# octavian-ganea/equidock_public

Hardware: NVIDIA H100
Metric: protein_pairs_per_sec_iegmn_fwd_kabsch (higher is better)
Workload: dtype f32

## Files before the change

### equidock_public_b200/_native.py

```python
from __future__ import annotations

import ctypes as C
import os

_HERE = os.path.dirname(os.path.abspath(__file__))
LIB_PATH = os.environ.get('EQD_LIB_PATH') or os.path.join(_HERE, 'libeqd_iegmn.so')

ABI_VERSION = 15
EDGE_FEATS, N_RBF, HID, H0, H0_PAD, N_RES_TYPES, HEADS, TILE_ROWS = 27, 15, 64, 69, 72, 21, 50, 128
MAX_HEADS = 64
STATUS_SVD_DEGENERATE, STATUS_NAN, STATUS_DEGREE_OVERFLOW, STATUS_BAD_RESIDUE = 1, 2, 4, 8

_vp, _i32, _f32 = C.c_void_p, C.c_int32, C.c_float


class EqdGraph(C.Structure):
    _fields_ = [('n_pairs', _i32), ('n_nodes', _i32), ('n_lig_nodes', _i32), ('n_edges', _i32),
                ('n_lig_edges', _i32), ('max_in_degree', _i32),
                ('seg_ptr', _vp), ('row_ptr', _vp), ('col_src', _vp), ('edge_dst', _vp),
                ('he_lig', _vp), ('he_rec', _vp),
                ('n_node_tiles', _i32), ('node_tiles', _vp)]


class EqdLayerParams(C.Structure):
    _fields_ = [('dh', _i32), ('dhp', _i32),
                ('w_proj', _vp), ('b_proj', _vp), ('w_edge1', _vp), ('edge_ln_g', _vp), ('edge_ln_b', _vp),
                ('w_edge2', _vp), ('b_edge2', _vp), ('w_coor1', _vp), ('b_coor1', _vp), ('w_coor2', _vp),
                ('b_coor2', _f32), ('w_edge_tc', _vp), ('w_node_tc', _vp), ('w_proj_tc', _vp),
                ('w_node1', _vp), ('b_node1', _vp), ('node_ln_g', _vp), ('node_ln_b', _vp),
                ('w_node2', _vp), ('b_node2', _vp),
                ('skip_weight_h', _f32), ('x_connection_init', _f32), ('leaky_slope', _f32), ('mma_products', _i32)]


class EqdLayerConsts(C.Structure):
    _fields_ = [('edge', _f32 * 64 * 5), ('node', _f32 * 304), ('proj_bias', _f32 * 320)]


class EqdDropout(C.Structure):
    _fields_ = [('seed', C.c_uint64), ('p', _f32), ('scale', _f32), ('threshold', C.c_uint32), ('layer', _i32),
                ('rank', _i32), ('reserved', _i32)]


def dropout_descriptor(p: float, seed: int, layer: int, rank: int = 0) -> EqdDropout:
    import numpy as np
    d = EqdDropout()
    d.seed, d.p, d.layer, d.rank = int(seed) & 0xFFFFFFFFFFFFFFFF, float(p), int(layer), int(rank)
    d.threshold = min(int(round(float(p) * 2.0 ** 32)), 0xFFFFFFFF)
    d.scale = 0.0 if p >= 1.0 else float(np.float32(1.0 / (1.0 - float(p))))
    return d


class EqdLayerNorms(C.Structure):
    _fields_ = [('coors_ln_g', _vp), ('coors_ln_b', _vp), ('final_ln_g', _vp), ('final_ln_b', _vp)]


class EqdLayer(C.Structure):
    _fields_ = [('dev', EqdLayerParams), ('consts', EqdLayerConsts), ('dropout', EqdDropout), ('norms', EqdLayerNorms)]


class EqdForwardIO(C.Structure):
    _fields_ = [(n, _vp) for n in ('emb', 'res_lig', 'res_rec', 'mu_lig', 'mu_rec', 'x_lig', 'x_rec', 'rot', 'trans',
                                   'ligand_out', 'sing', 'status', 'h_out', 'x_out', 'keypts', 'cov', 'ymean', 'stage_events',
                                   'train_stash')] + \
               [('train_stash_bytes', C.c_size_t)]


class EqdHeadParams(C.Structure):
    _fields_ = [('w_mean', _vp), ('b_mean', _vp), ('w_key', _vp), ('w_query', _vp), ('m_qk', _vp), ('leaky_slope', _f32),
                ('n_heads', _i32)]


class EqdPairArchive(C.Structure):
    _fields_ = [('n_pairs', _i32)] + [(n, _vp) for n in (
        'lig_node_ptr', 'rec_node_ptr', 'lig_edge_ptr', 'rec_edge_ptr', 'pocket_ptr', 'lig_res_feat', 'rec_res_feat',
        'lig_x', 'rec_x', 'lig_mu_r_norm', 'rec_mu_r_norm', 'lig_src', 'lig_dst', 'rec_src', 'rec_dst', 'lig_he', 'rec_he',
        'lig_new_x', 'pocket_coors', 'bound_lig', 'bound_rec', 'lig_centroid')]


class EqdBatchOut(C.Structure):
    _fields_ = [(n, _vp) for n in ('res_feat', 'x', 'new_x', 'mu_r_norm', 'row_ptr', 'col_src', 'edge_dst', 'he_lig', 'he_rec',
                                   'seg_ptr',
                                   'node_tiles', 'pocket_ptr', 'pocket_lig', 'pocket_rec', 'bound_lig', 'bound_rec', 'rot',
                                   'trans')]


_G, _L, _H = C.POINTER(EqdGraph), C.POINTER(EqdLayer), C.POINTER(EqdHeadParams)
PROTOTYPES = {
    'eqd_abi_version': (C.c_int, []),
    'eqd_workspace_bytes': (C.c_size_t, [_i32, _i32, _i32]),
    'eqd_workspace_bytes_k': (C.c_size_t, [_i32, _i32, _i32, _i32]),
    'eqd_embed': (C.c_int, [_G, _vp, _vp, _vp, _vp, _vp, _vp, _vp, _vp, _vp, _vp]),
    'eqd_embed_checked': (C.c_int, [_G, _vp, _vp, _vp, _vp, _vp, _vp, _vp, _vp, _vp, _vp, _vp]),
    'eqd_project': (C.c_int, [_G, _L, _vp, _i32, _vp, _vp]),
    'eqd_edge_stage': (C.c_int, [_G, _L, _vp, _vp, _vp, _vp, _vp, _vp, _vp]),
    'eqd_edge_stage_ffma': (C.c_int, [_G, _L, _vp, _vp, _vp, _vp, _vp, _vp, _vp]),
    'eqd_node_stage': (C.c_int, [_G, _L, _L, _vp, _i32, _vp, _vp, _vp, _vp, _vp, _vp, _vp]),
    'eqd_kv_blocks_bytes': (C.c_size_t, [_i32]),
    'eqd_project_tc': (C.c_int, [_G, _L, _vp, _vp, _vp, _vp]),
    'eqd_project_tc0': (C.c_int, [_G, _L, _vp, _vp, _vp, _vp, _vp]),
    'eqd_attention_tc0': (C.c_int, [_G, _vp, _vp, _vp, _vp, _vp]),
    'eqd_node_mlp_tc0': (C.c_int, [_G, _L, _vp, _vp, _vp, _vp, _vp]),
    'eqd_node_stage_tc0': (C.c_int, [_G, _L, _L, _vp, _vp, _vp, _vp, _vp, _vp, _vp, _vp, _vp]),
    'eqd_kv_blocks': (C.c_int, [_G, _vp, _i32, _i32, _i32, _vp, _vp]),
    'eqd_attention_tc': (C.c_int, [_G, _vp, _vp, _vp, _vp]),
    'eqd_node_mlp_tc': (C.c_int, [_G, _L, _vp, _vp, _vp, _vp, _vp, _vp]),
    'eqd_node_stage_tc': (C.c_int, [_G, _L, _L, _vp, _vp, _vp, _vp, _vp, _vp, _vp, _vp, _vp]),
    'eqd_iegmn_layer_forward': (C.c_int, [_G, _L, _L, _vp, _i32, _vp, _vp, _vp, _vp, _vp, _vp, _vp, _vp, _vp, _vp,
                                          _vp]),
    'eqd_head_fold': (C.c_int, [_H, _vp, _vp]),
    'eqd_forward_workspace_bytes': (C.c_size_t, [_G]),
    'eqd_forward_workspace_bytes_k': (C.c_size_t, [_G, _i32]),
    'eqd_iegmn_forward': (C.c_int, [_G, C.POINTER(_L), _i32, _H, C.POINTER(EqdForwardIO), _vp, C.c_size_t, _vp]),
    'eqd_forward_stash_bytes': (C.c_size_t, [_G, _i32]),
    'eqd_forward_stash_offsets': (C.c_int, [_G, _i32, C.POINTER(C.c_size_t)]),
    'eqd_tn_partial_floats': (C.c_size_t, [C.c_int64, _i32, _i32, C.POINTER(_i32), C.POINTER(_i32)]),
    'eqd_tn_gemm': (C.c_int, [_vp, _i32, _i32, _vp, _i32, _i32, C.c_int64, _f32, _vp, _vp, C.POINTER(_i32), _vp]),
    'eqd_grad_reduce': (C.c_int, [_vp, _i32, C.c_int64, _vp, _vp, _i32, _vp, _vp]),
    'eqd_bwd_node_mlp': (C.c_int, [_G, _L] + [_vp] * 3 + [_i32, _vp, _vp, _i32] + [_vp] * 9 + [C.POINTER(_i32), _vp]),
    'eqd_bwd_attention': (C.c_int, [_G, _L, _vp, _vp, _i32, _vp, _vp, _vp, _vp]),
    'eqd_bwd_edge': (C.c_int, [_G, _L] + [_vp] * 14 + [C.POINTER(_i32), _vp]),
    'eqd_bwd_edge_gather': (C.c_int, [_G, _vp, _vp, _vp, _vp, _vp, _f32, _vp, _i32, _vp, _vp]),
    'eqd_bwd_project': (C.c_int, [_G, _L, _vp, _vp, _vp, _vp]),
    'eqd_bwd_embed': (C.c_int, [_G, _vp, _vp, _vp, _vp, _vp, _vp]),
    'eqd_bwd_head_workspace_bytes': (C.c_size_t, [_i32, _i32, _i32]),
    'eqd_bwd_head_workspace_bytes_k': (C.c_size_t, [_i32, _i32, _i32, _i32]),
    'eqd_bwd_head': (C.c_int, [_G, _H] + [_vp] * 9 + [C.c_size_t] + [_vp] * 6),
    'eqd_bwd_head_dropout': (C.c_int, [_G, _H, C.POINTER(EqdDropout)] + [_vp] * 9 + [C.c_size_t] + [_vp] * 6),
    'eqd_bwd_layer_inputs': (C.c_int, [_G, _L] + [_vp] * 5),
    'eqd_bwd_inputs': (C.c_int, [_G] + [_vp] * 11),
    'eqd_losses_workspace_bytes': (C.c_size_t, [_i32, _i32]),
    'eqd_losses': (C.c_int, [_G] + [_vp] * 7 + [_i32, _i32, _f32, _f32, _f32, _f32, _vp, C.c_size_t] + [_vp] * 6),
    'eqd_losses_workspace_bytes_k': (C.c_size_t, [_i32, _i32, _i32]),
    'eqd_losses_k': (C.c_int, [_G] + [_vp] * 4 + [_i32] + [_vp] * 3 + [_i32, _i32, _f32, _f32, _f32, _f32, _vp, C.c_size_t] +
                     [_vp] * 6),
    'eqd_graph_build_workspace_bytes': (C.c_size_t, [_i32]),
    'eqd_graph_build_knn': (C.c_int, [_i32, _i32, _i32, _vp, _vp, _vp, _vp, _vp, _f32, _i32, _vp, C.c_size_t, _vp, _vp, _vp, _vp]),
    'eqd_graph_build_edges': (C.c_int, [_i32, _vp, _vp, _vp, _vp, _vp, _vp, _vp]),
    'eqd_assemble_batch': (C.c_int, [C.POINTER(EqdPairArchive), _i32, _vp, _i32, C.c_uint64, C.c_uint64, _i32, _f32, _i32,
                                     C.POINTER(EqdBatchOut), _vp]),
    'eqd_rmsd_meter': (C.c_int, [_G, _vp, _vp, _vp, _vp, _vp, _vp]),
    'eqd_sqnorm_partials': (C.c_int, [_vp, C.c_int64, _vp, _i32, _vp]),
    'eqd_clip_adam': (C.c_int, [_vp, _vp, _vp, _vp, C.c_int64, _vp, _i32, _f32, _f32, _f32, _f32, _f32, _f32, _i32, _f32, _vp, _vp]),
    'eqd_event_create': (_vp, []),
    'eqd_event_destroy': (None, [_vp]),
    'eqd_event_elapsed_ms': (C.c_float, [_vp, _vp]),
    'eqd_keypoints': (C.c_int, [_G, _H, _vp, _vp, _vp, C.c_size_t, _vp, _vp, _vp, _vp]),
    'eqd_keypoints_dropout': (C.c_int, [_G, _H, C.POINTER(EqdDropout), _vp, _vp, _vp, C.c_size_t, _vp, _vp, _vp, _vp]),
    'eqd_kabsch_apply': (C.c_int, [_G, _vp, _vp, _vp, _vp, _vp, _vp, _vp, _vp, _vp, _vp]),
}

_lib = None


class NativeLibraryError(RuntimeError):
    pass


def load():
    global _lib
    if _lib is not None:
        return _lib
    if not os.path.isfile(LIB_PATH):
        raise NativeLibraryError(
            f'{LIB_PATH} not found: build it with equidock_public_b200/csrc/build.sh '
            '(python -c "import __graft_entry__ as g; g.build()"). This engine has no CPU fallback.')
    lib = C.CDLL(LIB_PATH)
    for name, (res, args) in PROTOTYPES.items():
        fn = getattr(lib, name)
        fn.restype, fn.argtypes = res, args
    if lib.eqd_abi_version() != ABI_VERSION:
        raise NativeLibraryError(f'ABI mismatch: library {lib.eqd_abi_version()} vs binding {ABI_VERSION}')
    _lib = lib
    return lib

# ... 15 lines not shown
```

### equidock_public_b200/csrc/attn_tc.cu

```cuda
#include "tc_common.cuh"

namespace eqd {

#define AT_THREADS 256
#define AT_KEYS 64
#define AT_CHUNK_BYTES 8192
#define AT_A_SPLIT 16384
#define AT_LD 68

struct AtGroupSmem {
  unsigned char k[2][3][AT_CHUNK_BYTES];
  unsigned char v[2][3][AT_CHUNK_BYTES];
  float red[EQD_TM * 2];
  float x5c[2][AT_KEYS * 16];
  float red5[EQD_TM * 2 * 5];
};
struct AtSmem {
  unsigned char qa[3 * AT_A_SPLIT];
  unsigned char pa[3 * AT_A_SPLIT];
  AtGroupSmem grp;
  unsigned long long k_bar[2], v_bar[2];
};

__global__ void __launch_bounds__(AT_THREADS, 1)
// ... 235 lines not shown
      m.j0 = __ldg(g.seg_ptr + pseg);
      m.j1 = __ldg(g.seg_ptr + pseg + 1);
      m.blk_lo = m.j0 >> 3;
      m.nchunks = (((m.j1 + 7) >> 3) - m.blk_lo + 7) >> 3;
      return k;
    }
    return -1;
  };
  unsigned kfill = 0, kcons = 0, vfill = 0, vcons = 0;
  auto fill = [&](unsigned char (*dst)[3][AT_CHUNK_BYTES], unsigned long long* bars, unsigned& n, const unsigned char* src,
                  int blk0) {
    if (t == 0) {
      unsigned long long* b = &bars[n & 1];
      mbar_expect_tx(b, 3 * AT_CHUNK_BYTES);
#pragma unroll
      for (int s = 0; s < 3; ++s) bulk_g2s(dst[n & 1][s], src + s * kv_split_stride + (long)blk0 * 1024, AT_CHUNK_BYTES, b);
    }
    ++n;
  };
  auto consume = [&](unsigned long long* bars, unsigned& n) {
    mbar_wait(&bars[n & 1], (n >> 1) & 1);
    return (int)((n++) & 1);
  };
  auto stage_q = [&](const AtTile& m) { stage_rows64(W.qs, proj, 320, 128, m.node0, m.nvalid, t); };

  const int fr0 = (t >> 5) * 16 + (lane >> 2), fc = 2 * (lane & 3);
  AtTile cur, nxt;
  int kt = find_tile(0, cur);
  bool k_ahead = false, v_ahead = false;
  if (kt >= 0) stage_q(cur);
  while (kt >= 0) {
    int ktn = -1;
    bool looked = false;
    auto look_ahead = [&]() {
      if (looked) return;
      looked = true;
      ktn = find_tile(kt + 1, nxt);
      if (ktn >= 0) stage_q(nxt);
    };
    if (cur.nchunks > 0 && !k_ahead) fill(W.k, W.k_bar, kfill, k_g, cur.blk_lo);
    cp_async_wait<0>();
    wg_barrier(bar);
    unsigned qf[3][4][4];
    staged_rows_to_a_split3<P>(W.qs, t, qf);
    wg_barrier(bar);
    auto k_desc = [&](int kb_) {
      return [&, kb_](int sp, int kk) { return b_desc_ex(k_saddr + (kb_ * 3 + sp) * AT_CHUNK_BYTES + kk * 256, 128, 1024); };
    };
    float mx[2] = {-INFINITY, -INFINITY};
    for (int c = 0; c < cur.nchunks; ++c) {
      const int kb_ = consume(W.k_bar, kcons);
      fill(W.k, W.k_bar, kfill, k_g, cur.blk_lo + (c + 1 < cur.nchunks ? 8 * (c + 1) : 0));
      float s[32];
      wg_gemm6_rs_issue<64, 4, 0, true>(s, qf, k_desc(kb_), false);
      look_ahead();
      wg_mma_wait(s);
      const int key0 = (cur.blk_lo + 8 * c) * 8 + fc;
#pragma unroll
      for (int j = 0; j < 8; ++j)
#pragma unroll
        for (int e = 0; e < 2; ++e) {
          const int kn = key0 + 8 * j + e;
          const bool ok = kn >= cur.j0 && kn < cur.j1;
#pragma unroll
          for (int h = 0; h < 2; ++h) mx[h] = fmaxf(mx[h], ok ? s[4 * j + 2 * h + e] : -INFINITY);
        }
      wg_barrier(bar);
    }
    look_ahead();
#pragma unroll
    for (int h = 0; h < 2; ++h) {
      mx[h] = fmaxf(mx[h], __shfl_xor_sync(0xffffffffu, mx[h], 1));
      mx[h] = fmaxf(mx[h], __shfl_xor_sync(0xffffffffu, mx[h], 2));
    }
    float lh[2][2] = {{0.f, 0.f}, {0.f, 0.f}};
    float o_acc[32];
#pragma unroll
    for (int i = 0; i < 32; ++i) o_acc[i] = 0.f;
    if (cur.nchunks > 0 && !v_ahead) fill(W.v, W.v_bar, vfill, v_g, cur.blk_lo);
    for (int c = 0; c < cur.nchunks; ++c) {
      const int kb_ = consume(W.k_bar, kcons);
      const bool last = c + 1 == cur.nchunks;
      if (!last) {
        fill(W.k, W.k_bar, kfill, k_g, cur.blk_lo + 8 * (c + 1));
        fill(W.v, W.v_bar, vfill, v_g, cur.blk_lo + 8 * (c + 1));
      } else if (ktn >= 0 && nxt.nchunks > 0) {
        fill(W.k, W.k_bar, kfill, k_g, nxt.blk_lo);
        fill(W.v, W.v_bar, vfill, v_g, nxt.blk_lo);
      }
      float s[32];
      wg_gemm6_rs_issue<64, 4, 0, false, P>(s, qf, k_desc(kb_), false);
      wg_mma_wait(s);
      const int key0 = (cur.blk_lo + 8 * c) * 8 + fc;
#pragma unroll
      for (int j = 0; j < 8; ++j)
#pragma unroll
        for (int e = 0; e < 2; ++e) {
          const int kn = key0 + 8 * j + e;
          const bool ok = kn >= cur.j0 && kn < cur.j1;
#pragma unroll
          for (int h = 0; h < 2; ++h) {
            float& x = s[4 * j + 2 * h + e];
            x = ok ? expf(x - mx[h]) : 0.f;
          }
        }
      {
        float ps[32];
#pragma unroll
        for (int i = 0; i < 32; ++i) ps[i] = __shfl_xor_sync(0xffffffffu, s[i], 2);
#pragma unroll
        for (int h = 0; h < 2; ++h)
#pragma unroll
          for (int ch = 0; ch < 2; ++ch) {
            float s0 = 0.f, s1 = 0.f;
#pragma unroll
            for (int c4 = 0; c4 < 8; ++c4) {
              s0 = __fadd_rn(s0, chain_val(s, ps, h, ch, c4, 0));
              s1 = __fadd_rn(s1, chain_val(s, ps, h, ch, c4, 1));
            }
            const float sp = __fadd_rn(s0, s1);
            lh[h][ch] = __fadd_rn(lh[h][ch], __fadd_rn(sp, __shfl_xor_sync(0xffffffffu, sp, 1)));
          }
      }
      unsigned pf[3][4][4];
      acc_to_a_split3<4, P>(s, pf);
      const int vb_ = consume(W.v_bar, vcons);
      float o[32];
      wg_gemm6_rs_issue<64, 4, 1, false, P>(o, pf, [&](int sp, int kk) {
        return b_desc_ex(v_saddr + (vb_ * 3 + sp) * AT_CHUNK_BYTES + kk * 2048, 1024, 128); }, false);
      wg_mma_wait(o);
#pragma unroll
      for (int i = 0; i < 32; ++i) o_acc[i] = __fadd_rn(o_acc[i], o[i]);
      wg_barrier(bar);
    }
    k_ahead = v_ahead = ktn >= 0 && nxt.nchunks > 0 && cur.nchunks > 0;
#pragma unroll
    for (int h = 0; h < 2; ++h) {
      const float l = __fadd_rn(lh[h][0], lh[h][1]);
      const float inv = l > 0.f ? 1.f / l : 0.f;
      const int row = fr0 + 8 * h;
      if (row < cur.nvalid) {
        float* dst = mu + (long)(cur.node0 + row) * EQD_HID + fc;
#pragma unroll
        for (int j = 0; j < 8; ++j)
          *reinterpret_cast<float2*>(dst + 8 * j) = make_float2(o_acc[4 * j + 2 * h] * inv, o_acc[4 * j + 2 * h + 1] * inv);
      }
    }
    kt = ktn;
    cur = nxt;
  }
  cp_async_wait<0>();
}

template <int P>
static int launch_attention64_tc(const eqd_graph* g, const float* proj, const void* kv, float* mu, void* stream) {
  const size_t smem = AT_CHAINS * sizeof(AtChainSmem);
  EQD_SET_SMEM(attention64_tc_kernel<P>, smem);
  const int nht = 2 * g->n_node_tiles;
  int grid = (nht + AT_CHAINS - 1) / AT_CHAINS;
  if (grid > EQD_SMS) grid = EQD_SMS;
  const long split_stride = (long)((g->n_nodes + 7) / 8 + 8) * 1024;
  attention64_tc_kernel<P><<<grid, AT_CHAINS * 128, smem, (cudaStream_t)stream>>>(
      *g, proj, reinterpret_cast<const unsigned char*>(kv), split_stride, mu);
  EQD_CUDA_LAUNCH_CHECK();
  return EQD_OK;
}

}

int eqd_attention_tc_products(const eqd_graph* g, const float* proj, const void* kv, float* mu, int products, void* stream) {
  if (!g || !proj || !kv || !mu) return EQD_ERR_BAD_ARG;
  if (reinterpret_cast<uintptr_t>(kv) & 15) return EQD_ERR_BAD_ARG;
  if (products != 6 && products != 3) return EQD_ERR_UNSUPPORTED;
  if (g->n_node_tiles <= 0) return EQD_OK;
  return products == 3 ? eqd::launch_attention64_tc<3>(g, proj, kv, mu, stream)
                       : eqd::launch_attention64_tc<6>(g, proj, kv, mu, stream);
}

extern "C" int eqd_attention_tc(const eqd_graph* g, const float* proj, const void* kv, float* mu, void* stream) {
  return eqd_attention_tc_products(g, proj, kv, mu, 6, stream);
}

extern "C" int eqd_attention_tc0(const eqd_graph* g, const float* proj, const void* kv, const float* x5, float* mu,
                                 void* stream) {
  if (!g || !proj || !kv || !x5 || !mu) return EQD_ERR_BAD_ARG;
  if ((reinterpret_cast<uintptr_t>(kv) | reinterpret_cast<uintptr_t>(x5)) & 15) return EQD_ERR_BAD_ARG;
  if (g->n_node_tiles <= 0) return EQD_OK;
  const size_t smem = sizeof(eqd::AtSmem) + 128;
  EQD_SET_SMEM(eqd::attention0_tc_kernel, smem);
  const int grid = g->n_node_tiles < EQD_SMS ? g->n_node_tiles : EQD_SMS;
  const long split_stride = (long)((g->n_nodes + 7) / 8 + 8) * 1024;
  eqd::attention0_tc_kernel<<<grid, AT_THREADS, smem, (cudaStream_t)stream>>>(
      *g, proj, 128 + 3 * 72, reinterpret_cast<const unsigned char*>(kv), split_stride, x5, mu, EQD_H0_PAD);
  EQD_CUDA_LAUNCH_CHECK();
  return EQD_OK;
}
```

### equidock_public_b200/engine.py

```python
from __future__ import annotations

import ctypes as C
import sys
import threading
from typing import Dict, List, Optional, Sequence

import numpy as np
import torch

from . import _native as nat
from .hetero_graph import LIGAND, LL, RECEPTOR, RR


def _dev_f32(t, device):
    return t.detach().to(device=device, dtype=torch.float32).contiguous()


def _host_f32(t):
    return t.detach().to(device='cpu', dtype=torch.float32).contiguous()


def _upload_blob(tensors: Dict[str, torch.Tensor], device) -> Dict[str, torch.Tensor]:
    offs, total = {}, 0
    for k, t in tensors.items():
# ... 128 lines not shown
            w5p[:69, 80:144] = w5[:, 69:133]
            w5p[:69, 144:213] = w5[:, 133:202]
            tc['w_node_tc'] = torch.cat([umma_bf16x3(w5p), umma_bf16x3(p80(w6).contiguous())]).contiguous()
            assert tc['w_proj_tc'].numel() * 2 == 161280 and tc['w_node_tc'].numel() * 2 == 138240
            p80v = lambda v: torch.cat([v, z(80 - v.shape[0])])
            self.node_consts_host = torch.cat([p80v(b5), p80v(f('node_mlp.3.weight')), p80v(f('node_mlp.3.bias')), b6]).cpu().contiguous()
            pb = z(320)
            pb[64:128] = b1
            self.proj_bias_host = pb.cpu().contiguous()
        self.t = _upload_blob({
            **tc,
            'w_proj': w_proj, 'b_proj': b_proj, 'w_edge1': w_edge1,
            'edge_ln_g': f('edge_mlp.3.weight'), 'edge_ln_b': f('edge_mlp.3.bias'),
            'w_edge2': f('edge_mlp.4.weight').t().contiguous(), 'b_edge2': f('edge_mlp.4.bias'),
            'w_coor1': f('coors_mlp.0.weight').t().contiguous(), 'b_coor1': f('coors_mlp.0.bias'),
            'w_coor2': f('coors_mlp.4.weight').reshape(-1).contiguous(),
            'w_node1': w_node1, 'b_node1': pad(b5),
            'node_ln_g': pad(f('node_mlp.3.weight')), 'node_ln_b': pad(f('node_mlp.3.bias')),
            'w_node2': w_node2, 'b_node2': b6, 'w_edge_tc': w_edge_tc,
            **({'_coors_ln_g': f('coors_mlp.3.weight'), '_coors_ln_b': f('coors_mlp.3.bias')}
               if layer_norm_coors == 'LN' else {}),
            **({'_final_ln_g': f('final_h_layernorm_layer.weight'), '_final_ln_b': f('final_h_layernorm_layer.bias')}
               if final_h_layer_norm == 'LN' else {}),
        }, device)
        lay = nat.EqdLayer()
        s = lay.dev
        s.dh, s.dhp = dh, dhp
        for k, v in self.t.items():
            if not k.startswith('_'):
                setattr(s, k, v.data_ptr())
        for name, host in (('edge', self.edge_consts_host), ('node', self.node_consts_host), ('proj_bias', self.proj_bias_host)):
            if host is not None:
                flat = host.reshape(-1).numpy()
                C.memmove(C.addressof(getattr(lay.consts, name)), flat.ctypes.data, flat.nbytes)
        s.b_coor2 = float(sd['coors_mlp.4.bias'].detach().reshape(-1)[0].item())
        s.skip_weight_h, s.x_connection_init, s.leaky_slope = skip_weight_h, x_connection_init, leaky_slope
        if layer_norm_coors == 'LN':
            lay.norms.coors_ln_g, lay.norms.coors_ln_b = self.t['_coors_ln_g'].data_ptr(), self.t['_coors_ln_b'].data_ptr()
        if final_h_layer_norm == 'LN':
            lay.norms.final_ln_g, lay.norms.final_ln_b = self.t['_final_ln_g'].data_ptr(), self.t['_final_ln_b'].data_ptr()
        self.struct = lay
        self._descriptors = {}

    def descriptor(self, mma_products: int = 0):
        if mma_products == 0 or self.dh != nat.HID:
            return self.struct
        src, d = self._descriptors.get(mma_products, (None, None))
        if src is not self.struct:
            d = nat.EqdLayer.from_buffer_copy(self.struct)
            d.dev.mma_products = mma_products
            self._descriptors[mma_products] = (self.struct, d)
        return d


class PackedHead:

    def __init__(self, w_mean, b_mean, w_key, w_query, device, leaky_slope: float):
        dev = torch.device(device)
        inplace = all(t.is_cuda and t.device == dev and t.dtype == torch.float32 and t.is_contiguous() and t.data_ptr() % 16 == 0
                      for t in (b_mean, w_key, w_query)) and w_mean.is_cuda
        if inplace:
            self.t = {'w_mean': w_mean.detach().to(torch.float32).t().contiguous(), 'b_mean': b_mean.detach(),
                      'w_key': w_key.detach(), 'w_query': w_query.detach()}
        else:
            self.t = _upload_blob({'w_mean': _host_f32(w_mean).t().contiguous(), 'b_mean': _host_f32(b_mean),
                                   'w_key': _host_f32(w_key), 'w_query': _host_f32(w_query)}, device)
        self.n_heads = self.t['w_key'].shape[0] // nat.HID
        assert 1 <= self.n_heads <= nat.MAX_HEADS and self.t['w_key'].shape == (self.n_heads * nat.HID, nat.HID)
        assert self.t['w_query'].shape == self.t['w_key'].shape
        s = nat.EqdHeadParams()
        for k, v in self.t.items():
            if not k.startswith('_'):
                setattr(s, k, v.data_ptr())
        s.leaky_slope = leaky_slope
        s.n_heads = self.n_heads
        self.struct = s
        self.m_qk = torch.empty(self.n_heads, nat.HID, nat.HID, dtype=torch.float64, device=device)
        with torch.cuda.device(device):
            nat.check(nat.load().eqd_head_fold(C.byref(s), self.m_qk.data_ptr(), torch.cuda.current_stream().cuda_stream),
                      'eqd_head_fold')
        s.m_qk = self.m_qk.data_ptr()


def _aligned_he(he, device):
    he = he.to(device=device, dtype=torch.float32).contiguous()
    nbytes = he.numel() * 4
    try:
        room = he.untyped_storage().nbytes() - he.storage_offset() * 4
    except RuntimeError:
        room = nbytes
    if he.data_ptr() % 16 == 0 and room >= ((nbytes + 15) & ~15):
        return he
    buf = torch.empty(((nbytes + 15) // 16) * 4 + 4, dtype=torch.float32, device=device)
    own = buf[:he.numel()].view(he.shape)
    own.copy_(he)
    return own


def node_tiles_for(n_lig: Sequence[int], n_rec: Sequence[int], device):
    seg = np.zeros(len(n_lig) + len(n_rec) + 1, dtype=np.int64)
    seg[1:] = np.cumsum(np.asarray(list(n_lig) + list(n_rec), dtype=np.int64))
    tiles = [(s, n0) for s in range(len(seg) - 1) for n0 in range(int(seg[s]), int(seg[s + 1]), nat.TILE_ROWS)]
    small = torch.from_numpy(np.concatenate([seg.astype(np.int32), np.asarray(tiles, dtype=np.int32).reshape(-1)]))
    small = small.to(device, non_blocking=True)
    return seg, small[:len(seg)], small[len(seg):]


class GraphPlan:

    def __init__(self, n_lig: Sequence[int], n_rec: Sequence[int], src_l, dst_l, src_r, dst_r, he_l, he_r,
                 device, max_in_degree: int = 10):
        assert len(n_lig) == len(n_rec) and len(n_lig) > 0
        N_l = sum(int(v) for v in n_lig)
        N = N_l + sum(int(v) for v in n_rec)
        i32 = dict(dtype=torch.int32, device=device)
        src_l, dst_l = src_l.to(**i32), dst_l.to(**i32)
        src_r, dst_r = src_r.to(**i32), dst_r.to(**i32)
        E_l, E = int(src_l.shape[0]), int(src_l.shape[0]) + int(src_r.shape[0])
        col_src = torch.cat([src_l, src_r + N_l]).contiguous()
        edge_dst = torch.cat([dst_l, dst_r + N_l]).contiguous()
        d64 = edge_dst.long()
        unsorted = (d64[1:] < d64[:-1]).any() if E > 1 else None
        row_ptr = torch.searchsorted(edge_dst, torch.arange(N + 1, **i32), out_int32=True).contiguous()
        he_l, he_r = _aligned_he(he_l, device), _aligned_he(he_r, device)
        assert he_l.shape == (E_l, nat.EDGE_FEATS) and he_r.shape == (E - E_l, nat.EDGE_FEATS)
        self._finish(n_lig, n_rec, E_l, E, E_l, col_src, edge_dst, row_ptr, he_l, he_r, *node_tiles_for(n_lig, n_rec, device),
                     device, max_in_degree, unsorted)

    def _finish(self, n_lig, n_rec, E_l, E, n_lig_edges, col_src, edge_dst, row_ptr, he_l, he_r, seg_ptr_host, seg_ptr,
                node_tiles, device, max_in_degree, unsorted=None, keep=()):
        self.n_pairs = len(n_lig)
        self.forward_ws_bytes = {}
        self.n_lig_list, self.n_rec_list = [int(v) for v in n_lig], [int(v) for v in n_rec]
        self.N_l, self.N_r = sum(self.n_lig_list), sum(self.n_rec_list)
        self.N = self.N_l + self.N_r
        self.device = device
        self.E_l, self.E_r, self.E = int(E_l), int(E) - int(E_l), int(E)
        self.col_src, self.edge_dst, self.row_ptr = col_src, edge_dst, row_ptr
        self.unsorted = unsorted if unsorted is not None else torch.zeros((), dtype=torch.bool, device=device)
        self.unsorted_i32 = self.unsorted.to(torch.int32).reshape(1)
        self._arange = None
        self.he_l, self.he_r = he_l, he_r
        self.edge_perm = None
        self.seg_ptr_host, self.seg_ptr, self.node_tiles = seg_ptr_host, seg_ptr, node_tiles
        self.n_node_tiles = int(node_tiles.numel()) // 2
        self._keep = keep
        g = nat.EqdGraph()
        g.n_pairs, g.n_nodes, g.n_lig_nodes = self.n_pairs, self.N, self.N_l
        g.n_edges, g.n_lig_edges, g.max_in_degree = self.E, int(n_lig_edges), int(max_in_degree)
        g.seg_ptr, g.row_ptr = seg_ptr.data_ptr(), row_ptr.data_ptr()
        g.col_src, g.edge_dst = col_src.data_ptr(), edge_dst.data_ptr()
        g.he_lig, g.he_rec = he_l.data_ptr(), he_r.data_ptr()
        g.n_node_tiles, g.node_tiles = self.n_node_tiles, node_tiles.data_ptr()
        self.struct = g

    def refresh(self, graph) -> bool:
        n_l = [int(v) for v in graph.batch_num_nodes(LIGAND).tolist()]
        n_r = [int(v) for v in graph.batch_num_nodes(RECEPTOR).tolist()]
        src_l, dst_l = graph.edges(etype=LL)
        src_r, dst_r = graph.edges(etype=RR)
        if (n_l != self.n_lig_list or n_r != self.n_rec_list or int(src_l.shape[0]) != self.E_l
                or int(src_r.shape[0]) != self.E_r):
            return False
        E_l = self.E_l
        self.col_src[:E_l].copy_(src_l)
        torch.add(src_r, self.N_l, out=self.col_src[E_l:])
        self.edge_dst[:E_l].copy_(dst_l)
        torch.add(dst_r, self.N_l, out=self.edge_dst[E_l:])
        if self.E > 1:
            torch.any(self.edge_dst[1:] < self.edge_dst[:-1], dim=0, keepdim=True, out=self.unsorted.view(1))
        self.unsorted_i32.copy_(self.unsorted.view(1))
        if self._arange is None:
            self._arange = torch.arange(self.N + 1, dtype=torch.int32, device=self.device)
        torch.searchsorted(self.edge_dst, self._arange, out_int32=True, out=self.row_ptr)
        for own, new in ((self.he_l, graph.edges[LL].data['he']), (self.he_r, graph.edges[RR].data['he'])):
            if own.data_ptr() != new.data_ptr():
                own.copy_(new)
        return True

    @classmethod
    def from_device_arrays(cls, n_lig: Sequence[int], n_rec: Sequence[int], E_l: int, E: int, col_src, edge_dst, row_ptr,
                           he_l, he_r, seg_ptr, node_tiles, seg_ptr_host, device, max_in_degree: int = 10, keep=()) -> 'GraphPlan':
        plan = object.__new__(cls)
        plan._finish(n_lig, n_rec, E_l, E, E if he_r is he_l else E_l, col_src, edge_dst, row_ptr, he_l, he_r, seg_ptr_host,
                     seg_ptr, node_tiles, device, max_in_degree, keep=keep)
        return plan

    @classmethod
    def from_graph(cls, graph, device, max_in_degree: int = 10, he=None, sort: bool = False) -> 'GraphPlan':
        n_l = graph.batch_num_nodes(LIGAND).tolist()
        n_r = graph.batch_num_nodes(RECEPTOR).tolist()
        he_l, he_r = he if he is not None else (graph.edges[LL].data['he'], graph.edges[RR].data['he'])
        sides = [(*graph.edges(etype=LL), he_l), (*graph.edges(etype=RR), he_r)]
        perms = None
        if sort:
            sides = [tuple(t.to(device) for t in side) for side in sides]
            perms = tuple(torch.sort(d.long(), stable=True).indices for _, d, _ in sides)
            sides = [tuple(t[perm] for t in side) for side, perm in zip(sides, perms)]
        (src_l, dst_l, he_l), (src_r, dst_r, he_r) = sides
        plan = cls(n_l, n_r, src_l, dst_l, src_r, dst_r, he_l, he_r, device, max_in_degree)
        plan.edge_perm = perms
        return plan

    def caller_edge_order(self, dhe):
        dhe_l, dhe_r = dhe[:self.E_l], dhe[self.E_l:self.E]
        if self.edge_perm is not None:
            dhe_l = torch.empty_like(dhe_l).index_copy_(0, self.edge_perm[0].to(dhe.device), dhe_l)
            dhe_r = torch.empty_like(dhe_r).index_copy_(0, self.edge_perm[1].to(dhe.device), dhe_r)
        return dhe_l, dhe_r


def plan_for(graph, device, max_in_degree, sort: bool = False) -> GraphPlan:
    cached = getattr(graph, '_eqd_plan', None)
    if not sort and cached is not None and cached.device == device and cached.struct.max_in_degree == max_in_degree:
        return cached
    plan = GraphPlan.from_graph(graph, device, max_in_degree, sort=sort)
    try:
        graph._eqd_plan = plan
    except AttributeError:
        pass
    return plan


def retry_sorted(graph, plan: GraphPlan, run):
    try:
        return run(plan)
    except UnsortedEdges:
        return run(plan_for(graph, plan.device, plan.struct.max_in_degree, sort=True))


class _StatusPool:

    def __init__(self):
        self.free, self.lock = [], threading.Lock()

    def take(self, n: int) -> torch.Tensor:
        with self.lock:
            for i, b in enumerate(self.free):
                if b.numel() >= n:
                    return self.free.pop(i)
        return torch.empty(max(n, 1024), dtype=torch.int32, pin_memory=True)

    def give(self, buf: torch.Tensor):
        with self.lock:
            if len(self.free) < 64:
                self.free.append(buf)


_STATUS_POOL = _StatusPool()


class _StatusLease:

    def __init__(self, n):
        self.buf, self.n = _STATUS_POOL.take(n), n

    def view(self):
        return self.buf[:self.n]

    def release(self):
        if self.buf is not None:
            _STATUS_POOL.give(self.buf)
            self.buf = None

    def __del__(self):
        try:
            self.release()
        except Exception:
            pass


class NativeStageTimer:

    def __init__(self):
        self.lib, self.sets, self.spare = nat.load(), [], []

    def reserve(self, n_forwards, n_layers):
        for _ in range(n_forwards):
            self.spare.append((C.c_void_p * (4 * n_layers))(*[self.lib.eqd_event_create() for _ in range(4 * n_layers)]))

    def new_forward(self, n_layers):
        if self.spare and len(self.spare[-1]) == 4 * n_layers:
            arr = self.spare.pop()
        else:
            arr = (C.c_void_p * (4 * n_layers))(*[self.lib.eqd_event_create() for _ in range(4 * n_layers)])
        self.sets.append(arr)
        return arr

    def _pairs(self, name):
        off = 0 if name == 'edge_stage' else 2
        for arr in self.sets:
            for li in range(len(arr) // 4):
                yield arr[li * 4 + off], arr[li * 4 + off + 1]

    def mean_ms(self, name):
        v = [self.lib.eqd_event_elapsed_ms(a, b) for a, b in self._pairs(name)]
        v = [x for x in v if x >= 0]
        return float(np.mean(v)) if v else None

    def total_ms(self, name):
        return float(sum(x for x in (self.lib.eqd_event_elapsed_ms(a, b) for a, b in self._pairs(name)) if x >= 0))

    def close(self):
        for arr in self.sets + self.spare:
            for e in arr:
                self.lib.eqd_event_destroy(e)
# ... 158 lines not shown
```

### include/eqd_iegmn.h

```cpp
#ifndef EQD_IEGMN_H
#define EQD_IEGMN_H

#include <stddef.h>
#include <stdint.h>

#ifdef __cplusplus
extern "C" {
#endif

#define EQD_ABI_VERSION 15

#define EQD_EDGE_FEATS 27
#define EQD_N_RBF 15
#define EQD_HID 64
#define EQD_H0 69
#define EQD_H0_PAD 72
#define EQD_N_RES_TYPES 21
#define EQD_HEADS 50
#define EQD_MAX_HEADS 64
#define EQD_TILE_ROWS 128

enum {
  EQD_OK = 0,
  EQD_ERR_BAD_ARG = -1,
  EQD_ERR_UNSUPPORTED = -2,
  EQD_ERR_WORKSPACE = -3
};

#define EQD_STATUS_SVD_DEGENERATE 1
#define EQD_STATUS_NAN 2
#define EQD_STATUS_DEGREE_OVERFLOW 4
#define EQD_STATUS_BAD_RESIDUE 8

typedef struct eqd_graph {
  int32_t n_pairs;
  int32_t n_nodes;
  int32_t n_lig_nodes;
  int32_t n_edges;
  int32_t n_lig_edges;
  int32_t max_in_degree;
  const int32_t* seg_ptr;
  const int32_t* row_ptr;
  const int32_t* col_src;
  const int32_t* edge_dst;
  const float* he_lig;
  const float* he_rec;
  int32_t n_node_tiles;
  const int32_t* node_tiles;
} eqd_graph;

typedef struct eqd_layer_params {
  int32_t dh, dhp;
  const float* w_proj;
  const float* b_proj;
  const float* w_edge1;
  const float* edge_ln_g;
  const float* edge_ln_b;
  const float* w_edge2;
  const float* b_edge2;
  const float* w_coor1;
  const float* b_coor1;
  const float* w_coor2;
  float b_coor2;
  const void* w_edge_tc;
  const void* w_node_tc;
  const void* w_proj_tc;
  const float* w_node1;
  const float* b_node1;
  const float* node_ln_g;
  const float* node_ln_b;
  const float* w_node2;
  const float* b_node2;
  float skip_weight_h;
  float x_connection_init;
  float leaky_slope;
  int32_t mma_products;
} eqd_layer_params;

typedef struct eqd_layer_consts {
  float edge[5][64];
  float node[304];
  float proj_bias[320];
} eqd_layer_consts;

typedef struct eqd_dropout {
  uint64_t seed;
  float p;
  float scale;
  uint32_t threshold;
  int32_t layer;
  int32_t rank;
  int32_t reserved;
} eqd_dropout;

typedef struct eqd_layer_norms {
  const float* coors_ln_g;
  const float* coors_ln_b;
  const float* final_ln_g;
  const float* final_ln_b;
} eqd_layer_norms;

typedef struct eqd_layer {
  eqd_layer_params dev;
  eqd_layer_consts consts;
  eqd_dropout dropout;
  eqd_layer_norms norms;
} eqd_layer;

typedef struct eqd_head_params {
  const float* w_mean;
  const float* b_mean;
  const float* w_key;
  const float* w_query;
  const double* m_qk;
  float leaky_slope;
  int32_t n_heads;
} eqd_head_params;

int eqd_abi_version(void);

size_t eqd_workspace_bytes(int32_t n_nodes, int32_t n_node_tiles, int32_t n_pairs);
size_t eqd_workspace_bytes_k(int32_t n_nodes, int32_t n_node_tiles, int32_t n_pairs, int32_t n_heads);

int eqd_embed(const eqd_graph* g, const float* emb ,
              const float* res_feat_lig, const float* res_feat_rec,
              const float* mu_lig, const float* mu_rec,
              const float* x_lig , const float* x_rec ,
              float* h0, double* x64, void* stream);
int eqd_embed_checked(const eqd_graph* g, const float* emb, const float* res_feat_lig, const float* res_feat_rec,
                      const float* mu_lig, const float* mu_rec, const float* x_lig, const float* x_rec,
                      float* h0, double* x64, int32_t* status , void* stream);

int eqd_project(const eqd_graph* g, const eqd_layer* p, const float* h, int32_t ldh,
                float* proj, void* stream);

int eqd_edge_stage(const eqd_graph* g, const eqd_layer* p, const float* proj,
                   const double* x_in, const double* x_orig, float* aggr, double* x_out,
                   int32_t* status , void* stream);

int eqd_edge_stage_ffma(const eqd_graph* g, const eqd_layer* p, const float* proj,
                        const double* x_in, const double* x_orig, float* aggr, double* x_out,
                        int32_t* status , void* stream);

int eqd_node_stage(const eqd_graph* g, const eqd_layer* p, const eqd_layer* p_next,
                   const float* h_in, int32_t ldh, const float* h0, const float* proj,
                   const float* aggr, float* mu, float* h_out, float* proj_next, void* stream);

size_t eqd_kv_blocks_bytes(int32_t n_nodes);
int eqd_project_tc(const eqd_graph* g, const eqd_layer* p, const float* h , float* proj,
                   void* kv, void* stream);
int eqd_project_tc0(const eqd_graph* g, const eqd_layer* p, const float* h0 , float* proj ,
                    void* kv, float* x5 , void* stream);
int eqd_kv_blocks(const eqd_graph* g, const float* proj, int32_t pw, int32_t koff, int32_t voff, void* kv,
                  void* stream);
int eqd_attention_tc(const eqd_graph* g, const float* proj, const void* kv, float* mu, void* stream);
int eqd_node_mlp_tc(const eqd_graph* g, const eqd_layer* p, const float* h_in, const float* aggr,
                    const float* mu, const float* h0, float* h_out, void* stream);
int eqd_node_stage_tc(const eqd_graph* g, const eqd_layer* p, const eqd_layer* p_next,
                      const float* h_in, const float* h0, const float* proj, const float* aggr, void* kv,
                      float* mu, float* h_out, float* proj_next, void* stream);

int eqd_attention_tc0(const eqd_graph* g, const float* proj , const void* kv, const float* x5 ,
                      float* mu , void* stream);
int eqd_node_mlp_tc0(const eqd_graph* g, const eqd_layer* p, const float* h0 , const float* aggr,
                     const float* mu , float* h_out , void* stream);
int eqd_node_stage_tc0(const eqd_graph* g, const eqd_layer* p, const eqd_layer* p_next, const float* h0,
                       const float* proj, const float* aggr, void* kv, const float* x5, float* mu, float* h_out,
                       float* proj_next, void* stream);

int eqd_iegmn_layer_forward(const eqd_graph* g, const eqd_layer* p, const eqd_layer* p_next,
                            const float* h_in, int32_t ldh, const float* h0,
                            const double* x_in, const double* x_orig,
                            float* proj, float* proj_next, float* aggr, float* mu,
                            float* h_out, double* x_out, int32_t* status, void* stream);

int eqd_head_fold(const eqd_head_params* hp, double* m_qk , void* stream);

int eqd_keypoints(const eqd_graph* g, const eqd_head_params* hp, const float* h ,
                  const double* x , void* workspace, size_t workspace_bytes,
                  double* keypts, double* ymean, double* cov, void* stream);
int eqd_keypoints_dropout(const eqd_graph* g, const eqd_head_params* hp, const eqd_dropout* dropout, const float* h,
                          const double* x, void* workspace, size_t workspace_bytes, double* keypts, double* ymean,
                          double* cov, void* stream);

int eqd_kabsch_apply(const eqd_graph* g, const double* cov, const double* ymean, const float* x_lig_in,
                     const int32_t* pair_mask, float* rot, float* trans, float* ligand_out,
                     double* sing, int32_t* status, void* stream);


typedef struct eqd_forward_io {
  const float* emb;
  const float* res_lig;
  const float* res_rec;
  const float* mu_lig;
  const float* mu_rec;
  const float* x_lig;
  const float* x_rec;
  float* rot;
  float* trans;
  float* ligand_out;
// ... 156 lines not shown
```

Before: 42570.

## Add segment-resident cross-attention kernel keeping partner K/V planes in shared memory

Adds an attention kernel that assigns one protein segment per CTA and loads the partner segment's full K/V split planes into shared memory once via bulk async copies. All query tiles of that segment then reuse those planes, with a two-pass softmax (max pass, then exp/sum and PV pass). This replaces the streaming per-chunk K/V pipeline when every segment fits within 248 nodes. The goal is to cut repeated K/V global loads and pipeline overhead. The trade-offs are extra score-GEMM work from the two passes, a grid capped at the number of segments, and a new graph struct field that changes the ABI layout.

```diff
diff --git a/equidock_public_b200/_native.py b/equidock_public_b200/_native.py
--- a/equidock_public_b200/_native.py
+++ b/equidock_public_b200/_native.py
@@ -19,7 +19,7 @@
                 ('n_lig_edges', _i32), ('max_in_degree', _i32),
                 ('seg_ptr', _vp), ('row_ptr', _vp), ('col_src', _vp), ('edge_dst', _vp),
                 ('he_lig', _vp), ('he_rec', _vp),
-                ('n_node_tiles', _i32), ('node_tiles', _vp)]
+                ('n_node_tiles', _i32), ('max_segment_nodes', _i32), ('node_tiles', _vp)]
 
 
 class EqdLayerParams(C.Structure):
diff --git a/equidock_public_b200/csrc/attn_tc.cu b/equidock_public_b200/csrc/attn_tc.cu
--- a/equidock_public_b200/csrc/attn_tc.cu
+++ b/equidock_public_b200/csrc/attn_tc.cu
@@ -411,14 +411,203 @@
   cp_async_wait<0>();
 }
 
+#define AT_RES_CHUNKS 4
+#define AT_RES_BLOCKS (AT_RES_CHUNKS * 8)
+#define AT_RES_PLANE (AT_RES_CHUNKS * AT_CHUNK_BYTES)
+#define AT_RES_MAX_NODES (8 * (AT_RES_BLOCKS - 1))
+
+struct __align__(128) AtResSmem {
+  unsigned char k[3][AT_RES_PLANE];
+  unsigned char v[3][AT_RES_PLANE];
+  float qs[AT_CHAINS][64 * 64];
+  unsigned long long res_k0, res_kv[AT_RES_CHUNKS];
+};
+static_assert(sizeof(AtResSmem) <= 227 * 1024, "resident K / V planes + Q staging exceed the 227 KB of shared memory per CTA");
+
+template <int P>
+__global__ void __launch_bounds__(AT_CHAINS * 128, 1)
+attention64_res_kernel(eqd_graph g, const float* __restrict__ proj, const unsigned char* __restrict__ kv,
+                       long kv_split_stride, float* __restrict__ mu) {
+  extern __shared__ __align__(128) unsigned char smem_raw[];
+  AtResSmem& R = *reinterpret_cast<AtResSmem*>(smem_raw);
+  const int tid = threadIdx.x, wgi = tid >> 7, t = tid & 127, lane = t & 31;
+  const int bar = 1 + wgi;
+  float* const qs = R.qs[wgi];
+  if (tid == 0) {
+    mbar_init(&R.res_k0, 1);
+    for (int c = 0; c < AT_RES_CHUNKS; ++c) mbar_init(&R.res_kv[c], 1);
+    asm volatile("fence.mbarrier_init.release.cluster;" ::: "memory");
+  }
+  __syncthreads();
+  const unsigned k_saddr = smem_u32(R.k), v_saddr = smem_u32(R.v);
+  const int B = g.n_pairs, nseg = 2 * B;
+  const unsigned char* k_g = kv;
+  const unsigned char* v_g = kv + 3 * kv_split_stride;
+
+  auto next_tile = [&](int& seg, int& h) {
+    for (; seg < nseg; seg += gridDim.x, h = wgi)
+      if (64 * h < __ldg(g.seg_ptr + seg + 1) - __ldg(g.seg_ptr + seg)) return;
+    seg = -1;
+  };
+  auto stage_q = [&](int seg, int h) {
+    const int node0 = __ldg(g.seg_ptr + seg) + 64 * h;
+    stage_rows64(qs, proj, 320, 128, node0, min(64, __ldg(g.seg_ptr + seg + 1) - node0), t);
+  };
+  int qseg = blockIdx.x, qh = wgi;
+  next_tile(qseg, qh);
+  if (qseg >= 0) stage_q(qseg, qh);
+
+  const int fr0 = (t >> 5) * 16 + (lane >> 2), fc = 2 * (lane & 3);
+  unsigned phase = 0;
+  for (int seg = blockIdx.x; seg < nseg; seg += gridDim.x) {
+    const int i0 = __ldg(g.seg_ptr + seg), i1 = __ldg(g.seg_ptr + seg + 1);
+    if (i1 <= i0) continue;
+    const int pseg = seg < B ? seg + B : seg - B;
+    const int j0 = __ldg(g.seg_ptr + pseg), j1 = __ldg(g.seg_ptr + pseg + 1);
+    const int blk_lo = j0 >> 3, nchunks = (((j1 + 7) >> 3) - blk_lo + 7) >> 3;
+    const bool fits = nchunks <= AT_RES_CHUNKS;
+    if (tid == 0 && fits) {
+      mbar_expect_tx(&R.res_k0, nchunks * AT_CHUNK_BYTES);
+      if (nchunks > 0) bulk_g2s(R.k[0], k_g + (long)blk_lo * 1024, nchunks * AT_CHUNK_BYTES, &R.res_k0);
+      for (int c = 0; c < AT_RES_CHUNKS; ++c) {
+        unsigned long long* b = &R.res_kv[c];
+        if (c >= nchunks) {
+          mbar_expect_tx(b, 0);
+          continue;
+        }
+        mbar_expect_tx(b, 5 * AT_CHUNK_BYTES);
+        const long off = (long)(blk_lo + 8 * c) * 1024;
+#pragma unroll
+        for (int s = 0; s < 3; ++s) {
+          if (s > 0) bulk_g2s(R.k[s] + c * AT_CHUNK_BYTES, k_g + s * kv_split_stride + off, AT_CHUNK_BYTES, b);
+          bulk_g2s(R.v[s] + c * AT_CHUNK_BYTES, v_g + s * kv_split_stride + off, AT_CHUNK_BYTES, b);
+        }
+      }
+    }
+    for (int h = wgi; 64 * h < i1 - i0; h += 2) {
+      const int node0 = i0 + 64 * h, nvalid = min(64, i1 - node0);
+      cp_async_wait<0>();
+      wg_barrier(bar);
+      unsigned qf[3][4][4];
+      staged_rows_to_a_split3<P>(qs, t, qf);
+      wg_barrier(bar);
+      qh += 2;
+      next_tile(qseg, qh);
+      if (qseg >= 0) stage_q(qseg, qh);
+      if (!fits) {
+        for (int i = t; i < nvalid * EQD_HID; i += 128) mu[(long)node0 * EQD_HID + i] = __int_as_float(0x7fc00000);
+        continue;
+      }
+      auto k_desc = [&](int c) {
+        return [&, c](int sp, int kk) { return b_desc_ex(k_saddr + sp * AT_RES_PLANE + c * AT_CHUNK_BYTES + kk * 256, 128, 1024); };
+      };
+      float mx[2] = {-INFINITY, -INFINITY};
+      if (nchunks > 0) mbar_wait(&R.res_k0, phase);
+      for (int c = 0; c < nchunks; ++c) {
+        float s[32];
+        wg_gemm6_rs_issue<64, 4, 0, true>(s, qf, k_desc(c), false);
+        wg_mma_wait(s);
+        const int key0 = (blk_lo + 8 * c) * 8 + fc;
+#pragma unroll
+        for (int j = 0; j < 8; ++j)
+#pragma unroll
+          for (int e = 0; e < 2; ++e) {
+            const int kn = key0 + 8 * j + e;
+            const bool ok = kn >= j0 && kn < j1;
+#pragma unroll
+            for (int hh = 0; hh < 2; ++hh) mx[hh] = fmaxf(mx[hh], ok ? s[4 * j + 2 * hh + e] : -INFINITY);
+          }
+      }
+#pragma unroll
+      for (int hh = 0; hh < 2; ++hh) {
+        mx[hh] = fmaxf(mx[hh], __shfl_xor_sync(0xffffffffu, mx[hh], 1));
+        mx[hh] = fmaxf(mx[hh], __shfl_xor_sync(0xffffffffu, mx[hh], 2));
+      }
+      float lh[2][2] = {{0.f, 0.f}, {0.f, 0.f}};
+      float o_acc[32];
+#pragma unroll
+      for (int i = 0; i < 32; ++i) o_acc[i] = 0.f;
+      for (int c = 0; c < nchunks; ++c) {
+        mbar_wait(&R.res_kv[c], phase);
+        float s[32];
+        wg_gemm6_rs_issue<64, 4, 0, false, P>(s, qf, k_desc(c), false);
+        wg_mma_wait(s);
+        const int key0 = (blk_lo + 8 * c) * 8 + fc;
+#pragma unroll
+        for (int j = 0; j < 8; ++j)
+#pragma unroll
+          for (int e = 0; e < 2; ++e) {
+            const int kn = key0 + 8 * j + e;
+            const bool ok = kn >= j0 && kn < j1;
+#pragma unroll
+            for (int hh = 0; hh < 2; ++hh) {
+              float& x = s[4 * j + 2 * hh + e];
+              x = ok ? expf(x - mx[hh]) : 0.f;
+            }
+          }
+        {
+          float ps[32];
+#pragma unroll
+          for (int i = 0; i < 32; ++i) ps[i] = __shfl_xor_sync(0xffffffffu, s[i], 2);
+#pragma unroll
+          for (int hh = 0; hh < 2; ++hh)
+#pragma unroll
+            for (int ch = 0; ch < 2; ++ch) {
+              float s0 = 0.f, s1 = 0.f;
+#pragma unroll
+              for (int c4 = 0; c4 < 8; ++c4) {
+                s0 = __fadd_rn(s0, chain_val(s, ps, hh, ch, c4, 0));
+                s1 = __fadd_rn(s1, chain_val(s, ps, hh, ch, c4, 1));
+              }
+              const float sp = __fadd_rn(s0, s1);
+              lh[hh][ch] = __fadd_rn(lh[hh][ch], __fadd_rn(sp, __shfl_xor_sync(0xffffffffu, sp, 1)));
+            }
+        }
+        unsigned pf[3][4][4];
+        acc_to_a_split3<4, P>(s, pf);
+        float o[32];
+        wg_gemm6_rs_issue<64, 4, 1, false, P>(o, pf, [&](int sp, int kk) {
+          return b_desc_ex(v_saddr + sp * AT_RES_PLANE + c * AT_CHUNK_BYTES + kk * 2048, 1024, 128); }, false);
+        wg_mma_wait(o);
+#pragma unroll
+        for (int i = 0; i < 32; ++i) o_acc[i] = __fadd_rn(o_acc[i], o[i]);
+      }
+#pragma unroll
+      for (int hh = 0; hh < 2; ++hh) {
+        const float l = __fadd_rn(lh[hh][0], lh[hh][1]);
+        const float inv = l > 0.f ? 1.f / l : 0.f;
+        const int row = fr0 + 8 * hh;
+        if (row < nvalid) {
+          float* dst = mu + (long)(node0 + row) * EQD_HID + fc;
+#pragma unroll
+          for (int j = 0; j < 8; ++j)
+            *reinterpret_cast<float2*>(dst + 8 * j) = make_float2(o_acc[4 * j + 2 * hh] * inv, o_acc[4 * j + 2 * hh + 1] * inv);
+        }
+      }
+    }
+    __syncthreads();
+    if (fits) phase ^= 1;
+  }
+  cp_async_wait<0>();
+}
+
 template <int P>
 static int launch_attention64_tc(const eqd_graph* g, const float* proj, const void* kv, float* mu, void* stream) {
+  const long split_stride = (long)((g->n_nodes + 7) / 8 + 8) * 1024;
+  if (g->max_segment_nodes > 0 && g->max_segment_nodes <= AT_RES_MAX_NODES) {
+    const size_t smem = sizeof(AtResSmem);
+    EQD_SET_SMEM(attention64_res_kernel<P>, smem);
+    const int grid = 2 * g->n_pairs < EQD_SMS ? 2 * g->n_pairs : EQD_SMS;
+    attention64_res_kernel<P><<<grid, AT_CHAINS * 128, smem, (cudaStream_t)stream>>>(
+        *g, proj, reinterpret_cast<const unsigned char*>(kv), split_stride, mu);
+    EQD_CUDA_LAUNCH_CHECK();
+    return EQD_OK;
+  }
   const size_t smem = AT_CHAINS * sizeof(AtChainSmem);
   EQD_SET_SMEM(attention64_tc_kernel<P>, smem);
   const int nht = 2 * g->n_node_tiles;
   int grid = (nht + AT_CHAINS - 1) / AT_CHAINS;
   if (grid > EQD_SMS) grid = EQD_SMS;
-  const long split_stride = (long)((g->n_nodes + 7) / 8 + 8) * 1024;
   attention64_tc_kernel<P><<<grid, AT_CHAINS * 128, smem, (cudaStream_t)stream>>>(
       *g, proj, reinterpret_cast<const unsigned char*>(kv), split_stride, mu);
   EQD_CUDA_LAUNCH_CHECK();
diff --git a/equidock_public_b200/engine.py b/equidock_public_b200/engine.py
--- a/equidock_public_b200/engine.py
+++ b/equidock_public_b200/engine.py
@@ -304,6 +304,7 @@
         g.col_src, g.edge_dst = col_src.data_ptr(), edge_dst.data_ptr()
         g.he_lig, g.he_rec = he_l.data_ptr(), he_r.data_ptr()
         g.n_node_tiles, g.node_tiles = self.n_node_tiles, node_tiles.data_ptr()
+        g.max_segment_nodes = max(self.n_lig_list + self.n_rec_list)
         self.struct = g
 
     def refresh(self, graph) -> bool:
diff --git a/include/eqd_iegmn.h b/include/eqd_iegmn.h
--- a/include/eqd_iegmn.h
+++ b/include/eqd_iegmn.h
@@ -46,6 +46,7 @@
   const float* he_lig;
   const float* he_rec;
   int32_t n_node_tiles;
+  int32_t max_segment_nodes;
   const int32_t* node_tiles;
 } eqd_graph;
 
```

After: 44490 (median of 6 runs). 4.5% higher.
